# yanmin-wu/EDA

Hardware: AMD Instinct MI355X
Metric: scenes/sec fwd+bwd (50k pts, 256 queries, 80 tok) (higher is better)
Workload: dtype f32

## Files before the change

eda_amd/csrc/capi.hip:

```cpp
#include "eda_common.h"

#include <stdarg.h>

int g_eda_fma_mode = 0;

static thread_local char g_err[512] = "";

void eda_set_error(const char *fmt, ...) {
  va_list ap;
  va_start(ap, fmt);
  vsnprintf(g_err, sizeof(g_err), fmt, ap);
  va_end(ap);
}

extern "C" int eda_version(void) { return EDA_HIP_ABI_VERSION; }
extern "C" const char *eda_last_error_string(void) { return g_err; }
extern "C" int eda_set_fma_mode(int mode) {
  if (mode != 0 && mode != 1) {
    eda_set_error("eda_set_fma_mode: mode must be 0 or 1");
    return EDA_ERR_INVALID_ARG;
  }
  g_eda_fma_mode = mode;
  return 0;
}
extern "C" int eda_get_fma_mode(void) { return g_eda_fma_mode; }

#include <atomic>
#include <mutex>
#include <stdlib.h>
namespace {
struct KnobRow { const char *name; long dflt; };
const KnobRow kKnobs[EDA_K_COUNT] = {
    {"EDA_FPS_CU_RESERVE", 0},
    {"EDA_FPS_BUCKET", -1},
    {"EDA_FPS_BUCKET_NW", 16},
    {"EDA_FPS_SMALL_T", 512},
    {"EDA_FPS_SPEC", 1},
    {"EDA_FPS_T", 512},
    {"EDA_FPS_P", -1},
    {"EDA_FPS_TEST_GIVEUP", 0},
    {"EDA_BQ_SCAN", 0},
    {"EDA_GEMM_DBG", 0},
    {"EDA_GEMM_DMA", -1},
    {"EDA_GEMM_DMA_MAP", -1},
    {"EDA_GEMM_STREAM_GRID", 0},
    {"EDA_GEMM_STREAM_B3", 1},
    {"EDA_GEMM_STREAM", 1},
    {"EDA_GEMM_STREAM_MINR", 32768},
    {"EDA_GEMM_CFG", -1},
    {"EDA_GEMM_LN_BM", 0},
    {"EDA_GEMM_LN_VAR", 0},
    {"EDA_GEMM_SPLITK", -1},
    {"EDA_GEMM_KC96", -1},
    {"EDA_GEMM_B3ROWS", 1},
    {"EDA_FPS_BACKGROUND", 0},
    {"EDA_MHA2_PRIO", 1},
    {"EDA_MHA2_BWD_DBUF", 0},
    {"EDA_MHA2_BWD_MERGE", -1},
    {"EDA_MHA2_KSPLIT", -1},
    {"EDA_MHA4", 0},
    {"EDA_MHA3", 1},
    {"EDA_MHA3_DBG", 0},
    {"EDA_BN_SMALL_CQ", 4},
    {"EDA_SA_LAYER_FUSE", 1},
    {"EDA_SA_BNBWD_FUSE", 1},
    {"EDA_SA_BWD_B3", 1},
    {"EDA_WGRAD_BF16X3", 1},
    {"EDA_WGRAD_WGS", 144},
    {"EDA_DETERMINISTIC", 0},
    {"EDA_FROZEN_NW", 0},
    {"EDA_PEER_SPIN_LOG2", 24},
    {"EDA_PEER_ALLOC", 0},
};
EdaEnv g_env;
std::atomic<int> g_env_ready{0};
std::atomic<unsigned> g_env_epoch{1};
std::mutex g_env_mu;
void env_load(EdaEnv &e) {
  for (int k = 0; k < EDA_K_COUNT; ++k) {
    const char *s = getenv(kKnobs[k].name);
    e.set[k] = s && *s;
    e.val[k] = e.set[k] ? atol(s) : kKnobs[k].dflt;
  }
  e.skip_on = false; e.skip_k = e.skip_n = 0; e.skip_e = -1;
  if (const char *sk = getenv("EDA_GEMM_STREAM_SKIP"))
    e.skip_on = sscanf(sk, "%d,%d,%d", &e.skip_k, &e.skip_n, &e.skip_e) >= 2;
}
}
int g_eda_deterministic = -1;
const EdaEnv &eda_env() {
  if (!g_env_ready.load(std::memory_order_acquire)) {
    std::lock_guard<std::mutex> lock(g_env_mu);
    if (!g_env_ready.load(std::memory_order_relaxed)) { env_load(g_env); g_env_ready.store(1, std::memory_order_release); }
  }
  return g_env;
}
unsigned eda_env_epoch() { return g_env_epoch.load(std::memory_order_relaxed); }
void eda_fps_env_reset();
void eda_gemm_env_reset();
void eda_wgrad_env_reset();
extern "C" int eda_reload_env(void) {
  {
    std::lock_guard<std::mutex> lock(g_env_mu);
    env_load(g_env);
    g_env_ready.store(1, std::memory_order_release);
    g_env_epoch.fetch_add(1, std::memory_order_relaxed);
  }
  g_eda_deterministic = -1;
  eda_fps_env_reset(); eda_gemm_env_reset(); eda_wgrad_env_reset();
  return 0;
}
extern "C" int eda_set_deterministic(int on) {
  if (on != 0 && on != 1) { eda_set_error("eda_set_deterministic: 0 or 1"); return EDA_ERR_INVALID_ARG; }
  g_eda_deterministic = on;
  return 0;
}
extern "C" int eda_get_deterministic(void) { return eda_deterministic() ? 1 : 0; }

namespace {
__global__ __launch_bounds__(256) void zero_kernel(uint4 *p16, size_t n16, unsigned char *tail, size_t ntail) {
  const size_t i = (size_t)blockIdx.x * 256 + threadIdx.x;
  const size_t stride = (size_t)gridDim.x * 256;
  for (size_t k = i; k < n16; k += stride) p16[k] = make_uint4(0u, 0u, 0u, 0u);
  if (i < ntail) tail[i] = 0;
}
}

int eda_zero_async(void *ptr, size_t bytes, hipStream_t stream) {
  if (bytes == 0) return 0;
  unsigned char *p = reinterpret_cast<unsigned char *>(ptr);
  size_t head = (16 - (reinterpret_cast<uintptr_t>(p) & 15u)) & 15u;
  if (head > bytes) head = bytes;
  if (head) {
    hipLaunchKernelGGL(zero_kernel, dim3(1), dim3(256), 0, stream, nullptr, (size_t)0, p, head);
    p += head; bytes -= head;
  }
  const size_t n16 = bytes / 16, ntail = bytes % 16;
  size_t blocks = (n16 + 255) / 256;
  if (blocks > 4096) blocks = 4096;
  if (blocks < 1) blocks = 1;
  hipLaunchKernelGGL(zero_kernel, dim3((unsigned)blocks), dim3(256), 0, stream,
                     reinterpret_cast<uint4 *>(p), n16, p + n16 * 16, ntail);
  hipError_t e = hipGetLastError();
  if (e != hipSuccess) { eda_set_error("eda_zero_async: %s", hipGetErrorString(e)); return (int)e; }
  return 0;
// ... 133 lines not shown
```

eda_amd/csrc/eda_common.h:

```cpp
#pragma once
#include <hip/hip_runtime.h>
#include <stdint.h>
#include <stdio.h>

#include "../../include/eda_hip.h"

#define EDA_WAVE 64

void eda_set_error(const char *fmt, ...);
extern int g_eda_fma_mode;

enum EdaKnob : int {
  EDA_K_FPS_CU_RESERVE, EDA_K_FPS_BUCKET, EDA_K_FPS_BUCKET_NW, EDA_K_FPS_SMALL_T, EDA_K_FPS_SPEC, EDA_K_FPS_T, EDA_K_FPS_P,
  EDA_K_FPS_TEST_GIVEUP, EDA_K_BQ_SCAN, EDA_K_GEMM_DBG, EDA_K_GEMM_DMA, EDA_K_GEMM_DMA_MAP, EDA_K_GEMM_STREAM_GRID,
  EDA_K_GEMM_STREAM_B3, EDA_K_GEMM_STREAM, EDA_K_GEMM_STREAM_MINR, EDA_K_GEMM_CFG, EDA_K_GEMM_LN_BM, EDA_K_GEMM_LN_VAR,
  EDA_K_GEMM_SPLITK, EDA_K_GEMM_KC96, EDA_K_GEMM_B3ROWS, EDA_K_FPS_BACKGROUND, EDA_K_MHA2_PRIO, EDA_K_MHA2_BWD_DBUF, EDA_K_MHA2_BWD_MERGE, EDA_K_MHA2_KSPLIT, EDA_K_MHA4, EDA_K_MHA3, EDA_K_MHA3_DBG, EDA_K_BN_SMALL_CQ, EDA_K_SA_LAYER_FUSE, EDA_K_SA_BNBWD_FUSE,
  EDA_K_SA_BWD_B3, EDA_K_WGRAD_BF16X3, EDA_K_WGRAD_WGS, EDA_K_DETERMINISTIC, EDA_K_FROZEN_NW, EDA_K_PEER_SPIN_LOG2, EDA_K_PEER_ALLOC, EDA_K_COUNT
};
struct EdaEnv {
  long val[EDA_K_COUNT];
  bool set[EDA_K_COUNT];
  int skip_k, skip_n, skip_e;
  bool skip_on;
};
const EdaEnv &eda_env();
unsigned eda_env_epoch();
static inline long eda_knob(EdaKnob k) { return eda_env().val[k]; }
static inline bool eda_knob_set(EdaKnob k) { return eda_env().set[k]; }
extern int g_eda_deterministic;
static inline bool eda_deterministic() { return (g_eda_deterministic < 0 ? eda_knob(EDA_K_DETERMINISTIC) : g_eda_deterministic) != 0; }

#define EDA_CHECK_ARG(cond, msg)                         \
  do {                                                   \
    if (!(cond)) {                                       \
      eda_set_error("%s: %s", __func__, msg);            \
      return EDA_ERR_INVALID_ARG;                        \
    }                                                    \
  } while (0)

#include <mutex>
#include <set>
#include <utility>
static inline hipError_t eda_set_max_dynamic_lds(const void *kern, size_t bytes) {
  static std::mutex mu;
  static std::set<std::pair<const void *, int>> done;
  int dev = 0;
  hipError_t e = hipGetDevice(&dev);
  if (e != hipSuccess) return e;
  std::lock_guard<std::mutex> lock(mu);
  if (done.count({kern, dev})) return hipSuccess;
  e = hipFuncSetAttribute(kern, hipFuncAttributeMaxDynamicSharedMemorySize, (int)bytes);
  if (e == hipSuccess) done.insert({kern, dev});
  return e;
}

#define EDA_CHECK_LAUNCH()                                              \
  do {                                                                  \
    hipError_t e__ = hipGetLastError();                                 \
    if (e__ != hipSuccess) {                                            \
      eda_set_error("%s: launch failed: %s", __func__,                  \
                    hipGetErrorString(e__));                            \
      return (int)e__;                                                  \
    }                                                                   \
  } while (0)

#define EDA_CHECK_HIP(expr)                                             \
  do {                                                                  \
    hipError_t e__ = (expr);                                            \
    if (e__ != hipSuccess) {                                            \
      eda_set_error("%s: %s failed: %s", __func__, #expr,               \
                    hipGetErrorString(e__));                            \
      return (int)e__;                                                  \
    }                                                                   \
  } while (0)

template <int MODE>
__device__ __forceinline__ float eda_sumsq3(float a, float b, float c) {
  if (MODE == 0) {
    float t = b * b;
    t = __builtin_fmaf(a, a, t);
    t = __builtin_fmaf(c, c, t);
    return t;
  } else {
    return (a * a + b * b) + c * c;
  }
}

#define EDA_DPP_QUAD_XOR1 0xB1
#define EDA_DPP_QUAD_XOR2 0x4E
#define EDA_DPP_ROW_ROR(n) (0x120 + (n))

template <int CTRL>
__device__ __forceinline__ int eda_dpp(int v) {
  return __builtin_amdgcn_update_dpp(v, v, CTRL, 0xF, 0xF, false);
}

__device__ __forceinline__ int eda_row_max_i32(int v) {
  v = max(v, eda_dpp<EDA_DPP_QUAD_XOR1>(v));
  v = max(v, eda_dpp<EDA_DPP_QUAD_XOR2>(v));
// ... 62 lines not shown
```

eda_amd/csrc/mha2.h:

```cpp
#pragma once
#include <hip/hip_runtime.h>

struct Mha2Args {
  const float *q, *k, *v;
  long q_sb, q_sl, k_sb, k_sl, v_sb, v_sl;
  float *o; long o_sb, o_sl;
  float *lse;
  const unsigned char *mask;
  int B, H, Lq, Lk;
  float scale, p_drop;
  const unsigned long long *seed_ptr; unsigned salt;
  const float *dout; long do_sb, do_sl;
  float *dq, *dk, *dv;
  long dq_sb, dq_sl, dk_sb, dk_sl, dv_sb, dv_sl;
  int n_kb;
  int n_qs;
  int q_per_wg;
  int prio_mode;
  int dtype;
  float *dq_part;
  float *dkv_part;
  int bwd_merge;
  unsigned *bwd_tickets;
  const float *xq; long xq_sb, xq_sl;
  const float *wq; long ldwq;
  const float *bq;
  float *q_out; long qo_sb, qo_sl;
  int n_ksplit, keys_per_split;
  int dbg3;
  float *fwd_part;
  unsigned *fwd_tickets;
};

int eda_mha2_fwd_launch(Mha2Args &a, void *ws, size_t ws_bytes, hipStream_t stream);
size_t eda_mha2_fwd_workspace_bytes(int B, int H, int Lq, int Lk);
int eda_mha3_fwd_launch(Mha2Args &a, hipStream_t stream);
bool eda_mha4_takes(int dtype, int Lq, int Lk);
size_t eda_mha4_fwd_workspace_bytes(int B, int H, int Lq, int Lk);
int eda_mha4_fwd_launch(Mha2Args &a, void *ws, size_t ws_bytes, hipStream_t stream);
int eda_mha2_qproj_fwd_launch(Mha2Args &a, hipStream_t stream);
int eda_mha2_bwd_launch(Mha2Args &a, void *ws, size_t ws_bytes, unsigned *tickets, size_t tickets_bytes, hipStream_t stream);
size_t eda_mha2_bwd_workspace_bytes(int B, int H, int Lq, int Lk);
size_t eda_mha2_bwd_ticket_bytes(int B, int H, int Lq, int Lk);
```

eda_amd/csrc/mha2.hip:

```cpp
#include "eda_common.h"
#include "mha2.h"

#include <stdlib.h>

namespace {

constexpr int HD = 36;
constexpr int KSTEPS = 9;
constexpr float LOG2E = 1.4426950408889634f;
constexpr float LN2 = 0.6931471805599453f;

typedef float f32x4 __attribute__((ext_vector_type(4)));
typedef unsigned u32x2 __attribute__((ext_vector_type(2)));

#ifdef EDA_MHA2_PROFILE
__device__ unsigned long long mha2_prof[64 * 8];
#define PSTAMP(slot)                                                   \
  do {                                                                 \
    __builtin_amdgcn_sched_barrier(0);                                 \
    const unsigned long long now__ = __builtin_amdgcn_s_memtime();     \
    asm volatile("s_waitcnt lgkmcnt(0)" ::"s"(now__));                 \
    prof_acc[slot] += now__ - prof_t;                                  \
    prof_t = now__;                                                    \
    __builtin_amdgcn_sched_barrier(0);                                 \
// ... 1172 lines not shown
      a.n_ksplit = sp.ns;
      const int chunks = (a.Lk + FWD_SPLIT_CHK - 1) / FWD_SPLIT_CHK;
      a.keys_per_split = (chunks + sp.ns - 1) / sp.ns * FWD_SPLIT_CHK;
      const bool one = a.keys_per_split == FWD_SPLIT_CHK;
      return one ? launch_fwd<4, 4, FWD_SPLIT_CHK, 1, true>(a, stream) : launch_fwd<4, 4, FWD_SPLIT_CHK, 2, true>(a, stream);
    }
  }
  {
    const int rc3 = eda_mha3_fwd_launch(a, stream);
    if (rc3 >= 0) return rc3;
  }
  const bool short_q = (long)BH * ((a.Lq + 255) / 256) < 192;
  if (a.Lk <= 144) {
    if (short_q) return launch_fwd<4, 2, 192, 1>(a, stream);
    return launch_fwd<16, 1, 192, 1>(a, stream);
  }
  if (a.Lk <= 256) {
    if (short_q) return launch_fwd<4, 4, 256, 1>(a, stream);
    return launch_fwd<16, 1, 256, 1>(a, stream);
  }
  if (short_q) return launch_fwd<4, 4, 256, 2>(a, stream);
  return launch_fwd<16, 1, 256, 2>(a, stream);
}

int eda_mha2_qproj_fwd_launch(Mha2Args &a, hipStream_t stream) {
  if (a.B == 0 || a.Lq == 0) return 0;
  const dim3 g((unsigned)(a.B * a.H * ((a.Lq + 63) / 64))), b(256);
  const bool drop = a.p_drop > 0.f;
#define EDA_QP(AR)                                                                                   \
  do {                                                                                               \
    if (drop) hipLaunchKernelGGL((mha2_qproj_fwd_kernel<true, AR>), g, b, 0, stream, a);             \
    else hipLaunchKernelGGL((mha2_qproj_fwd_kernel<false, AR>), g, b, 0, stream, a);                 \
  } while (0)
  if (a.dtype == EDA_DTYPE_BF16) EDA_QP(ArBf16);
  else if (a.dtype == EDA_DTYPE_F16) EDA_QP(ArFp16);
  else EDA_QP(ArF32);
#undef EDA_QP
  EDA_CHECK_LAUNCH();
  return 0;
}

#ifdef EDA_MHA2_PROFILE
extern "C" int eda_mha2_profile_read(unsigned long long *out16) {
  static unsigned long long all[64 * 8], zero[64 * 8];
  if (hipMemcpyFromSymbol(all, HIP_SYMBOL(mha2_prof), sizeof(all)) != hipSuccess) return 1;
  for (int i = 0; i < 16; ++i) out16[i] = 0;
  for (int s = 0; s < 64; ++s)
    for (int i = 0; i < 8; ++i) out16[i] += all[s * 8 + i];
  return hipMemcpyToSymbol(HIP_SYMBOL(mha2_prof), zero, sizeof(zero)) != hipSuccess;
}
#endif

size_t eda_mha2_bwd_ticket_bytes(int B, int H, int Lq, int Lk) {
  if (B <= 0 || Lq <= 0 || Lk <= 0) return 0;
  return (sizeof(unsigned) * bwd_ticket_words(bwd_plan(B, H, Lq, Lk), B, H) + 255) / 256 * 256;
}
size_t eda_mha2_bwd_workspace_bytes(int B, int H, int Lq, int Lk) {
  if (B <= 0 || Lq <= 0 || Lk <= 0) return 0;
  return eda_mha2_bwd_ticket_bytes(B, H, Lq, Lk) + sizeof(float) * bwd_workspace_floats(bwd_plan(B, H, Lq, Lk), B, H, Lq, Lk);
}

int eda_mha2_bwd_launch(Mha2Args &a, void *ws, size_t ws_bytes, unsigned *tickets, size_t tickets_bytes, hipStream_t stream) {
  if (a.B == 0) return 0;
  a.prio_mode = (int)eda_knob(EDA_K_MHA2_PRIO);
  const BwdPlan p = bwd_plan(a.B, a.H, a.Lq, a.Lk);
  a.n_kb = p.n_kb; a.n_qs = p.n_qs; a.q_per_wg = p.q_per_wg;
  const size_t tk = eda_mha2_bwd_ticket_bytes(a.B, a.H, a.Lq, a.Lk);
  const size_t need = tk + sizeof(float) * bwd_workspace_floats(p, a.B, a.H, a.Lq, a.Lk);
  EDA_CHECK_ARG(need == 0 || (ws && ws_bytes >= need && (reinterpret_cast<uintptr_t>(ws) & 15u) == 0),
                "workspace of eda_mha_bwd_workspace_bytes() required (16-byte aligned)");
  EDA_CHECK_ARG(!tickets || tickets_bytes >= tk, "ticket buffer of eda_mha_bwd_ticket_bytes() required");
  float *w = reinterpret_cast<float *>(reinterpret_cast<unsigned char *>(ws) + tk);
  a.dq_part = nullptr; a.dkv_part = nullptr; a.bwd_tickets = nullptr;
  if (p.n_kb > 1) { a.dq_part = w; w += (size_t)p.n_kb * a.B * a.Lq * a.H * HD; }
  if (p.n_qs > 1) a.dkv_part = w;
  if (tk) {
    a.bwd_tickets = tickets ? tickets : reinterpret_cast<unsigned *>(ws);
    if (!tickets)
      if (int rc = eda_zero_async(ws, tk, stream)) return rc;
  }
  a.bwd_merge = p.merge;
  const bool dbuf = eda_knob(EDA_K_MHA2_BWD_DBUF) != 0;
  int rc;
  if (p.variant == 0) rc = launch_bwd<16, 1, 64, 2>(a, stream);
  else if (p.variant == 1) rc = dbuf ? launch_bwd<9, 1, 64, 2>(a, stream) : launch_bwd<9, 1, 64, 1>(a, stream);
  else rc = dbuf ? launch_bwd<5, 3, 96, 2>(a, stream) : launch_bwd<5, 3, 96, 1>(a, stream);
  if (rc || p.merge) return rc;
  const int D = a.H * HD;
  if (p.n_kb > 1) {
    const long items = (long)a.B * a.Lq * D / 4;
    hipLaunchKernelGGL(mha2_part_reduce_kernel, dim3((unsigned)((items + 255) / 256)), dim3(256), 0, stream,
                       a.dq_part, p.n_kb, 1, a.B, a.Lq, D, a.dq, a.dq_sb, a.dq_sl, a.dq, a.dq_sb, a.dq_sl);
    EDA_CHECK_LAUNCH();
  }
  if (p.n_qs > 1) {
    const long items = 2L * a.B * a.Lk * D / 4;
    hipLaunchKernelGGL(mha2_part_reduce_kernel, dim3((unsigned)((items + 255) / 256)), dim3(256), 0, stream,
                       a.dkv_part, p.n_qs, 2, a.B, a.Lk, D, a.dk, a.dk_sb, a.dk_sl, a.dv, a.dv_sb, a.dv_sl);
    EDA_CHECK_LAUNCH();
  }
  return 0;
}

namespace {

bool mult4(long v) { return (v & 3) == 0; }
bool al16(const void *p) { return (reinterpret_cast<uintptr_t>(p) & 15u) == 0; }

__global__ __launch_bounds__(256) void mha2_fill_rows_kernel(float *__restrict__ o, long sb, long sl, int B, int L, int D,
                                                             float value) {
  const long i = (long)blockIdx.x * 256 + threadIdx.x;
  if (i >= (long)B * L * D) return;
  const long row = i / D;
  const int col = (int)(i - row * D);
  const long bb = row / L, l = row - bb * L;
  o[bb * sb + l * sl + col] = value;
}
int fill_rows(float *o, long sb, long sl, int B, int L, int D, float value, hipStream_t stream) {
  const long n = (long)B * L * D;
  if (n <= 0) return 0;
  hipLaunchKernelGGL(mha2_fill_rows_kernel, dim3((unsigned)((n + 255) / 256)), dim3(256), 0, stream, o, sb, sl, B, L, D, value);
  EDA_CHECK_LAUNCH();
  return 0;
}

}

extern "C" size_t eda_mha_fwd_workspace_bytes(int B, int H, int Lq, int Lk) { return eda_mha2_fwd_workspace_bytes(B, H, Lq, Lk); }

extern "C" int eda_mha_fwd(const float *q, const float *k, const float *v, long q_sb, long q_sl, long k_sb, long k_sl,
                           long v_sb, long v_sl, const unsigned char *key_padding_mask, int B, int H, int Lq, int Lk,
                           int head_dim, float scale, float p_drop, const unsigned long long *seed_ptr, unsigned salt,
                           float *out, float *lse, int dtype, void *stream_) {
  return eda_mha_fwd_ws(q, k, v, q_sb, q_sl, k_sb, k_sl, v_sb, v_sl, key_padding_mask, B, H, Lq, Lk, head_dim, scale, p_drop,
                        seed_ptr, salt, out, lse, dtype, nullptr, 0, stream_);
}

extern "C" int eda_mha_fwd_ws(const float *q, const float *k, const float *v, long q_sb, long q_sl, long k_sb, long k_sl,
                              long v_sb, long v_sl, const unsigned char *key_padding_mask, int B, int H, int Lq, int Lk,
                              int head_dim, float scale, float p_drop, const unsigned long long *seed_ptr, unsigned salt,
                              float *out, float *lse, int dtype, void *ws, size_t ws_bytes, void *stream_) {
  hipStream_t stream = (hipStream_t)stream_;
  EDA_CHECK_ARG(dtype == EDA_DTYPE_F32 || dtype == EDA_DTYPE_BF16 || dtype == EDA_DTYPE_F16,
                "dtype must be EDA_DTYPE_F32 / BF16 / F16");
  EDA_CHECK_ARG(head_dim == HD, "only head_dim 36 (d_model 288 / 8 heads) is built");
  EDA_CHECK_ARG(B >= 0 && H > 0 && Lq >= 0 && Lk >= 0, "bad dimension");
  if (B == 0 || Lq == 0) return 0;
  EDA_CHECK_ARG(q && k && v && out && lse, "null pointer");
  EDA_CHECK_ARG(p_drop >= 0.f && p_drop < 1.f && (p_drop == 0.f || seed_ptr), "bad dropout arguments");
  EDA_CHECK_ARG(mult4(q_sb) && mult4(q_sl) && mult4(k_sb) && mult4(k_sl) && mult4(v_sb) && mult4(v_sl) &&
                    al16(q) && al16(k) && al16(v) && al16(out),
                "rows must be 16-byte aligned");
  EDA_CHECK_ARG((long)B * H <= 65535, "B*H too large");
  if (Lk == 0) {
    if (int rc = fill_rows(out, (long)Lq * H * HD, (long)H * HD, B, Lq, H * HD, 0.f, stream)) return rc;
    return fill_rows(lse, (long)H * Lq, (long)Lq, B, H, Lq, -INFINITY, stream);
  }
  Mha2Args m = {};
  m.q = q; m.k = k; m.v = v; m.q_sb = q_sb; m.q_sl = q_sl; m.k_sb = k_sb; m.k_sl = k_sl;
  m.v_sb = v_sb; m.v_sl = v_sl; m.o = out; m.o_sb = (long)Lq * H * HD; m.o_sl = (long)H * HD;
  m.lse = lse; m.mask = key_padding_mask; m.B = B; m.H = H; m.Lq = Lq; m.Lk = Lk; m.scale = scale;
  m.p_drop = p_drop; m.seed_ptr = seed_ptr; m.salt = salt; m.dtype = dtype;
  return eda_mha2_fwd_launch(m, ws, ws_bytes, stream);
}

extern "C" int eda_mha_qproj_supported(int H, int head_dim, int Lk) { return H * head_dim == QP_D && head_dim == HD && Lk >= 1 && Lk <= 192; }

// ... 107 lines not shown
```

Measured before the change: 464.4.

## Add MFMA-based bf16x3 split-precision attention backward kernel for variant 0

Adds a new attention backward kernel (mha3_bwd) that splits f32 Q/K/V/dO into three bf16 planes and computes the score and gradient products with 16x16x32 bf16 MFMA using six-product emulation. It stages Q/dO/O chunks into LDS via global_load_lds and overlaps conversion of the next chunk with the dQ phase on separate waves. It is enabled by default for the variant-0 config and falls back to the old path when shapes do not fit. The aim is to replace the slower f32 backward, at the cost of bf16x3 precision emulation and heavy LDS use that limits occupancy.

After: 469.3, median of 6. 1.01x the previous value.

```diff
diff --git a/eda_amd/csrc/capi.hip b/eda_amd/csrc/capi.hip
--- a/eda_amd/csrc/capi.hip
+++ b/eda_amd/csrc/capi.hip
@@ -61,6 +61,7 @@
     {"EDA_MHA4", 0},
     {"EDA_MHA3", 1},
     {"EDA_MHA3_DBG", 0},
+    {"EDA_MHA3_BWD", 1},
     {"EDA_BN_SMALL_CQ", 4},
     {"EDA_SA_LAYER_FUSE", 1},
     {"EDA_SA_BNBWD_FUSE", 1},
diff --git a/eda_amd/csrc/eda_common.h b/eda_amd/csrc/eda_common.h
--- a/eda_amd/csrc/eda_common.h
+++ b/eda_amd/csrc/eda_common.h
@@ -14,7 +14,7 @@
   EDA_K_FPS_CU_RESERVE, EDA_K_FPS_BUCKET, EDA_K_FPS_BUCKET_NW, EDA_K_FPS_SMALL_T, EDA_K_FPS_SPEC, EDA_K_FPS_T, EDA_K_FPS_P,
   EDA_K_FPS_TEST_GIVEUP, EDA_K_BQ_SCAN, EDA_K_GEMM_DBG, EDA_K_GEMM_DMA, EDA_K_GEMM_DMA_MAP, EDA_K_GEMM_STREAM_GRID,
   EDA_K_GEMM_STREAM_B3, EDA_K_GEMM_STREAM, EDA_K_GEMM_STREAM_MINR, EDA_K_GEMM_CFG, EDA_K_GEMM_LN_BM, EDA_K_GEMM_LN_VAR,
-  EDA_K_GEMM_SPLITK, EDA_K_GEMM_KC96, EDA_K_GEMM_B3ROWS, EDA_K_FPS_BACKGROUND, EDA_K_MHA2_PRIO, EDA_K_MHA2_BWD_DBUF, EDA_K_MHA2_BWD_MERGE, EDA_K_MHA2_KSPLIT, EDA_K_MHA4, EDA_K_MHA3, EDA_K_MHA3_DBG, EDA_K_BN_SMALL_CQ, EDA_K_SA_LAYER_FUSE, EDA_K_SA_BNBWD_FUSE,
+  EDA_K_GEMM_SPLITK, EDA_K_GEMM_KC96, EDA_K_GEMM_B3ROWS, EDA_K_FPS_BACKGROUND, EDA_K_MHA2_PRIO, EDA_K_MHA2_BWD_DBUF, EDA_K_MHA2_BWD_MERGE, EDA_K_MHA2_KSPLIT, EDA_K_MHA4, EDA_K_MHA3, EDA_K_MHA3_DBG, EDA_K_MHA3_BWD, EDA_K_BN_SMALL_CQ, EDA_K_SA_LAYER_FUSE, EDA_K_SA_BNBWD_FUSE,
   EDA_K_SA_BWD_B3, EDA_K_WGRAD_BF16X3, EDA_K_WGRAD_WGS, EDA_K_DETERMINISTIC, EDA_K_FROZEN_NW, EDA_K_PEER_SPIN_LOG2, EDA_K_PEER_ALLOC, EDA_K_COUNT
 };
 struct EdaEnv {
diff --git a/eda_amd/csrc/mha2.h b/eda_amd/csrc/mha2.h
--- a/eda_amd/csrc/mha2.h
+++ b/eda_amd/csrc/mha2.h
@@ -39,6 +39,7 @@
 size_t eda_mha4_fwd_workspace_bytes(int B, int H, int Lq, int Lk);
 int eda_mha4_fwd_launch(Mha2Args &a, void *ws, size_t ws_bytes, hipStream_t stream);
 int eda_mha2_qproj_fwd_launch(Mha2Args &a, hipStream_t stream);
+int eda_mha3_bwd_launch(Mha2Args &a, hipStream_t stream);
 int eda_mha2_bwd_launch(Mha2Args &a, void *ws, size_t ws_bytes, unsigned *tickets, size_t tickets_bytes, hipStream_t stream);
 size_t eda_mha2_bwd_workspace_bytes(int B, int H, int Lq, int Lk);
 size_t eda_mha2_bwd_ticket_bytes(int B, int H, int Lq, int Lk);
diff --git a/eda_amd/csrc/mha2.hip b/eda_amd/csrc/mha2.hip
--- a/eda_amd/csrc/mha2.hip
+++ b/eda_amd/csrc/mha2.hip
@@ -1278,7 +1278,10 @@
   a.bwd_merge = p.merge;
   const bool dbuf = eda_knob(EDA_K_MHA2_BWD_DBUF) != 0;
   int rc;
-  if (p.variant == 0) rc = launch_bwd<16, 1, 64, 2>(a, stream);
+  if (p.variant == 0) {
+    rc = eda_mha3_bwd_launch(a, stream);
+    if (rc < 0) rc = launch_bwd<16, 1, 64, 2>(a, stream);
+  }
   else if (p.variant == 1) rc = dbuf ? launch_bwd<9, 1, 64, 2>(a, stream) : launch_bwd<9, 1, 64, 1>(a, stream);
   else rc = dbuf ? launch_bwd<5, 3, 96, 2>(a, stream) : launch_bwd<5, 3, 96, 1>(a, stream);
   if (rc || p.merge) return rc;
diff --git a/eda_amd/csrc/mha3_bwd.hip b/eda_amd/csrc/mha3_bwd.hip
--- /dev/null
+++ b/eda_amd/csrc/mha3_bwd.hip
@@ -0,0 +1,547 @@
+#include "eda_common.h"
+#include "mha2.h"
+
+namespace {
+
+constexpr int HD = 36;
+constexpr float LOG2E = 1.4426950408889634f;
+constexpr int NW = 16, NT = NW * 64;
+constexpr int KB = 16 * NW;
+constexpr int QC = 32;
+constexpr int KROW = 40;
+constexpr int KREM = 24;
+constexpr int TROW = QC + 8;
+constexpr int DROW = KB + 8;
+constexpr int NPB = 6;
+
+typedef float f32x4 __attribute__((ext_vector_type(4)));
+typedef float f32x2 __attribute__((ext_vector_type(2)));
+typedef __bf16 bf16x2 __attribute__((ext_vector_type(2)));
+typedef __bf16 bf16x8 __attribute__((ext_vector_type(8)));
+typedef unsigned u32x2 __attribute__((ext_vector_type(2)));
+typedef unsigned u32x4 __attribute__((ext_vector_type(4)));
+
+constexpr int STG_B = QC * HD * 4;
+constexpr int RP_B = QC * KROW * 2;
+constexpr int RR_B = QC * KREM * 2;
+constexpr int TP_B = 32 * TROW * 2;
+constexpr int TR_B = 16 * TROW * 2;
+constexpr int DP_B = QC * DROW * 2;
+constexpr int KP_B = 32 * DROW * 2;
+constexpr int KR_B = 16 * DROW * 2;
+constexpr int O_STG = 0;
+constexpr int O_QP = O_STG + 3 * STG_B, O_QR = O_QP + 3 * RP_B;
+constexpr int O_EP = O_QR + RR_B, O_ER = O_EP + 3 * RP_B;
+constexpr int O_QT = O_ER + RR_B, O_QTR = O_QT + 3 * TP_B;
+constexpr int O_ET = O_QTR + TR_B, O_ETR = O_ET + 3 * TP_B;
+constexpr int O_DS = O_ETR + TR_B;
+constexpr int O_KT = O_DS + 3 * DP_B, O_KTR = O_KT + 3 * KP_B;
+constexpr int O_LSE = O_KTR + KR_B, O_DEL = O_LSE + QC * 4;
+constexpr int LDS_BYTES = O_DEL + QC * 4;
+static_assert(LDS_BYTES <= 160 * 1024, "LDS budget");
+static_assert(O_QP % 16 == 0 && O_EP % 16 == 0 && O_QT % 16 == 0 && O_ET % 16 == 0 && O_DS % 16 == 0 && O_KT % 16 == 0 &&
+              O_KTR % 16 == 0 && O_QTR % 16 == 0 && O_ETR % 16 == 0 && O_QR % 16 == 0 && O_ER % 16 == 0, "alignment");
+
+__device__ __forceinline__ unsigned hash32(unsigned x) {
+  x ^= x >> 16; x *= 0x7feb352dU; x ^= x >> 15; x *= 0x846ca68bU; x ^= x >> 16;
+  return x;
+}
+__device__ __forceinline__ float grp_sum(float v) {
+  u32x2 r = __builtin_amdgcn_permlane32_swap(__float_as_uint(v), __float_as_uint(v), false, false);
+  v = __uint_as_float(r.x) + __uint_as_float(r.y);
+  r = __builtin_amdgcn_permlane16_swap(__float_as_uint(v), __float_as_uint(v), false, false);
+  return __uint_as_float(r.x) + __uint_as_float(r.y);
+}
+__device__ __forceinline__ f32x4 grp_sum4(f32x4 v) {
+  f32x4 r;
+  r[0] = grp_sum(v[0]); r[1] = grp_sum(v[1]); r[2] = grp_sum(v[2]); r[3] = grp_sum(v[3]);
+  return r;
+}
+
+__device__ __forceinline__ void split2(float a, float b, unsigned (&pl)[3]) {
+  const bf16x2 h = __builtin_convertvector(f32x2{a, b}, bf16x2);
+  pl[0] = __builtin_bit_cast(unsigned, h);
+  const float ra = a - (float)h[0], rb = b - (float)h[1];
+  const bf16x2 m = __builtin_convertvector(f32x2{ra, rb}, bf16x2);
+  pl[1] = __builtin_bit_cast(unsigned, m);
+  const bf16x2 l = __builtin_convertvector(f32x2{ra - (float)m[0], rb - (float)m[1]}, bf16x2);
+  pl[2] = __builtin_bit_cast(unsigned, l);
+}
+
+__device__ __forceinline__ f32x4 mma32(u32x4 a, u32x4 b, f32x4 c) {
+  return __builtin_amdgcn_mfma_f32_16x16x32_bf16(__builtin_bit_cast(bf16x8, a), __builtin_bit_cast(bf16x8, b), c, 0, 0, 0);
+}
+__device__ __forceinline__ f32x4 prod6(const u32x4 (&a)[3], const u32x4 (&b)[3], f32x4 acc) {
+  f32x4 s = mma32(a[1], b[1], f32x4{0, 0, 0, 0});
+  acc = mma32(a[0], b[2], acc);
+  s = mma32(a[2], b[0], s);
+  acc = mma32(a[1], b[0], acc);
+  s = mma32(a[0], b[1], s);
+  acc = mma32(a[0], b[0], acc);
+  return acc + s;
+}
+
+struct DropCfg { unsigned seed, thresh; float inv_keep; };
+
+__device__ __forceinline__ void row_planes(const float *row, float mul, bool valid, int g, u32x4 (&pl)[3], u32x4 &rem) {
+  float4 x = make_float4(0.f, 0.f, 0.f, 0.f), y = x, z = x;
+  if (valid) {
+    x = *reinterpret_cast<const float4 *>(row + 8 * g);
+    y = *reinterpret_cast<const float4 *>(row + 8 * g + 4);
+    z = *reinterpret_cast<const float4 *>(row + 32);
+  }
+  const float v8[8] = {x.x * mul, x.y * mul, x.z * mul, x.w * mul, y.x * mul, y.y * mul, y.z * mul, y.w * mul};
+#pragma unroll
+  for (int i = 0; i < 4; ++i) {
+    unsigned w[3];
+    split2(v8[2 * i], v8[2 * i + 1], w);
+#pragma unroll
+    for (int p = 0; p < 3; ++p) pl[p][i] = w[p];
+  }
+  unsigned r01[3], r23[3];
+  split2(z.x * mul, z.y * mul, r01);
+  split2(z.z * mul, z.w * mul, r23);
+  const int pb = g == 1 ? 2 : 1;
+  rem = g < 3 ? u32x4{r01[0], r23[0], r01[pb], r23[pb]} : u32x4{0u, 0u, 0u, 0u};
+}
+
+template <bool DROP>
+__global__ __launch_bounds__(NT) void mha3_bwd_kernel(const Mha2Args a) {
+  extern __shared__ __attribute__((aligned(16))) unsigned char smem[];
+  float *stg = reinterpret_cast<float *>(smem + O_STG);
+  float *lse_s = reinterpret_cast<float *>(smem + O_LSE);
+  float *del_s = reinterpret_cast<float *>(smem + O_DEL);
+
+  const int tid = threadIdx.x, lane = tid & 63;
+  const int wave = __builtin_amdgcn_readfirstlane(tid >> 6);
+  const int g = lane >> 4, c = lane & 15;
+  const int BH = a.B * a.H;
+  const int bh = (int)(blockIdx.x % (unsigned)BH);
+  const int rest = (int)(blockIdx.x / (unsigned)BH);
+  const int kb = rest % a.n_kb, qsp = rest / a.n_kb;
+  const int b = bh / a.H, h = bh - b * a.H;
+  const int ks = wave;
+
+  const int kblock0 = kb * KB;
+  const int key0 = kblock0 + 16 * ks;
+  const bool wave_live = key0 < a.Lk;
+  const int nks_live = min(NW, (a.Lk - kblock0 + 15) >> 4);
+  const int ki = key0 + c;
+  const bool kvalid = ki < a.Lk;
+  const bool kdead = !kvalid || (a.mask && a.mask[(long)b * a.Lk + (kvalid ? ki : 0)]);
+
+  DropCfg dc = {0u, 0u, 1.f};
+  if (DROP && a.p_drop > 0.f) {
+    dc.seed = hash32((unsigned)(*a.seed_ptr) * 0x9E3779B1u + a.salt);
+    dc.thresh = (unsigned)((double)a.p_drop * 65536.0 + 0.5);
+    dc.inv_keep = 1.f / (1.f - a.p_drop);
+  }
+
+  for (int i = tid; i < 3 * DP_B / 4; i += NT) reinterpret_cast<unsigned *>(smem + O_DS)[i] = 0u;
+  for (int i = tid; i < 4 * TROW / 2; i += NT) {
+    reinterpret_cast<unsigned *>(smem + O_QTR + 12 * TROW * 2)[i] = 0u;
+    reinterpret_cast<unsigned *>(smem + O_ETR + 12 * TROW * 2)[i] = 0u;
+  }
+  for (int i = tid; i < 4 * DROW / 2; i += NT) reinterpret_cast<unsigned *>(smem + O_KTR + 12 * DROW * 2)[i] = 0u;
+  const float *kbase = a.k + (long)b * a.k_sb + h * HD;
+  for (int i = tid; i < (KB / 2) * HD; i += NT) {
+    const int kq = i / HD, d = i - kq * HD;
+    const int k0 = kblock0 + 2 * kq;
+    const float x0 = k0 < a.Lk ? kbase[(long)k0 * a.k_sl + d] : 0.f;
+    const float x1 = k0 + 1 < a.Lk ? kbase[(long)(k0 + 1) * a.k_sl + d] : 0.f;
+    unsigned pl[3];
+    split2(x0, x1, pl);
+    if (d < 32) {
+#pragma unroll
+      for (int p = 0; p < 3; ++p) *reinterpret_cast<unsigned *>(smem + O_KT + p * KP_B + (d * DROW + 2 * kq) * 2) = pl[p];
+    } else {
+#pragma unroll
+      for (int p = 0; p < 3; ++p) *reinterpret_cast<unsigned *>(smem + O_KTR + ((4 * p + d - 32) * DROW + 2 * kq) * 2) = pl[p];
+    }
+  }
+  u32x4 kp[3], kx, vp[3], vx;
+  {
+    const int kr = min(ki, a.Lk - 1);
+    const bool ld = wave_live && kvalid;
+    row_planes(kbase + (long)kr * a.k_sl, 1.f, ld, g, kp, kx);
+    row_planes(a.v + (long)b * a.v_sb + (long)kr * a.v_sl + h * HD, dc.inv_keep, ld, g, vp, vx);
+  }
+
+  const int qbeg = qsp * a.q_per_wg;
+  const int qend = min(a.Lq, qbeg + a.q_per_wg);
+  const float *qbase = a.q + (long)b * a.q_sb + h * HD;
+  const float *dbase = a.dout + (long)b * a.do_sb + h * HD;
+  const float *obase = a.o + (long)b * a.o_sb + h * HD;
+  const float sl2 = a.scale * LOG2E;
+  const int D = a.H * HD;
+  float *dq_out = a.dq + (long)b * a.dq_sb + h * HD;
+  long dq_sl = a.dq_sl;
+  if (a.n_kb > 1) { dq_out = a.dq_part + ((long)kb * a.B + b) * a.Lq * D + h * HD; dq_sl = D; }
+  const __amdgpu_buffer_rsrc_t rs_dq = __builtin_amdgcn_make_buffer_rsrc(dq_out, 0, a.Lq * D * 4, 0x00020000);
+
+  auto stage = [&](int q0) {
+    constexpr int G = QC * 9, P = (G + 63) / 64;
+    for (int pc = wave; pc < 3 * P; pc += NW) {
+      const int t = pc / P, pp = pc - t * P;
+      const int i = 64 * pp + lane;
+      if (G % 64 == 0 || i < G) {
+        const int row = i / 9, c4 = i - row * 9;
+        const int grow = min(q0 + row, a.Lq - 1);
+        const float *src = t == 0 ? qbase + (long)grow * a.q_sl : (t == 1 ? dbase + (long)grow * a.do_sl : obase + (long)grow * a.o_sl);
+        __builtin_amdgcn_global_load_lds((const __attribute__((address_space(1))) void *)(src + 4 * c4),
+                                         (__attribute__((address_space(3))) void *)(stg + t * (QC * HD) + 256 * pp), 16, 0, 0);
+      }
+    }
+  };
+
+  auto convert = [&](int q0, int w0, int nw) {
+    const int nthr = 64 * nw;
+    int t0 = tid - 64 * w0;
+    asm volatile("" : "+v"(t0));
+    if (t0 < QC * 8) {
+      const int row = t0 >> 3, sub = t0 & 7;
+      const int gr = min(q0 + row, a.Lq - 1);
+      const float ls = a.lse[(long)bh * a.Lq + gr];
+      const float *dr = stg + QC * HD + row * HD, *orow = stg + 2 * QC * HD + row * HD;
+      const float4 d4 = *reinterpret_cast<const float4 *>(dr + 4 * sub), o4 = *reinterpret_cast<const float4 *>(orow + 4 * sub);
+      float part = d4.x * o4.x + d4.y * o4.y + d4.z * o4.z + d4.w * o4.w;
+      if (sub == 0) {
+        const float4 d8 = *reinterpret_cast<const float4 *>(dr + 32), o8 = *reinterpret_cast<const float4 *>(orow + 32);
+        part += d8.x * o8.x + d8.y * o8.y + d8.z * o8.z + d8.w * o8.w;
+      }
+      part += __shfl_xor(part, 1);
+      part += __shfl_xor(part, 2);
+      part += __shfl_xor(part, 4);
+      if (sub == 0) {
+        const bool valid = q0 + row < qend;
+        lse_s[row] = valid ? ls * LOG2E : INFINITY;
+        del_s[row] = valid ? part : 0.f;
+      }
+    }
+    for (int i = t0; i < 2 * (QC / 2) * 18; i += nthr) {
+      const int t = i / ((QC / 2) * 18), r = i - t * ((QC / 2) * 18);
+      const int qq = r / 18, dp = r - qq * 18;
+      const float *src = stg + t * (QC * HD) + 2 * qq * HD + 2 * dp;
+      const float2 x0 = *reinterpret_cast<const float2 *>(src), x1 = *reinterpret_cast<const float2 *>(src + HD);
+      unsigned pa[3], pb[3];
+      split2(x0.x, x0.y, pa);
+      split2(x1.x, x1.y, pb);
+      unsigned char *rp = smem + (t ? O_EP : O_QP), *rr = smem + (t ? O_ER : O_QR);
+      unsigned char *tp = smem + (t ? O_ET : O_QT), *tr = smem + (t ? O_ETR : O_QTR);
+      if (dp < 16) {
+#pragma unroll
+        for (int p = 0; p < 3; ++p) {
+          *reinterpret_cast<unsigned *>(rp + p * RP_B + ((2 * qq) * KROW + 2 * dp) * 2) = pa[p];
+          *reinterpret_cast<unsigned *>(rp + p * RP_B + ((2 * qq + 1) * KROW + 2 * dp) * 2) = pb[p];
+        }
+      } else {
+        const int o = dp - 16;
+        unsigned *r0 = reinterpret_cast<unsigned *>(rr + (2 * qq) * KREM * 2) + o;
+        unsigned *r1 = reinterpret_cast<unsigned *>(rr + (2 * qq + 1) * KREM * 2) + o;
+        r0[0] = pa[0]; r0[2] = pa[0]; r0[4] = pa[1]; r0[6] = pa[0]; r0[8] = pa[2]; r0[10] = pa[1];
+        r1[0] = pb[0]; r1[2] = pb[0]; r1[4] = pb[1]; r1[6] = pb[0]; r1[8] = pb[2]; r1[10] = pb[1];
+      }
+#pragma unroll
+      for (int p = 0; p < 3; ++p) {
+        const unsigned lo = (pa[p] & 0xffffu) | (pb[p] << 16);
+        const unsigned hi = (pa[p] >> 16) | (pb[p] & 0xffff0000u);
+        const int d = 2 * dp;
+        unsigned char *base = d < 32 ? tp + p * TP_B + d * TROW * 2 : tr + (4 * p + d - 32) * TROW * 2;
+        *reinterpret_cast<unsigned *>(base + 4 * qq) = lo;
+        *reinterpret_cast<unsigned *>(base + TROW * 2 + 4 * qq) = hi;
+      }
+    }
+  };
+
+  f32x4 dk[3] = {{0, 0, 0, 0}, {0, 0, 0, 0}, {0, 0, 0, 0}};
+  f32x4 dv[3] = {{0, 0, 0, 0}, {0, 0, 0, 0}, {0, 0, 0, 0}};
+
+  auto trow = [&](const unsigned char *p, int c, int g) {
+    const unsigned char *row = p + (c * TROW + 4 * g) * 2;
+    const u32x2 lo = *reinterpret_cast<const u32x2 *>(row), hi = *reinterpret_cast<const u32x2 *>(row + 32);
+    return u32x4{lo.x, lo.y, hi.x, hi.y};
+  };
+
+  auto phase_a = [&](int q0) {
+    if (!wave_live) return;
+    int ln = lane;
+    asm volatile("" : "+v"(ln));
+    const int c = ln & 15, g = ln >> 4;
+    const int nsub = min(2, (qend - q0 + 15) >> 4);
+    float pd[2][4], ds[2][4];
+#pragma unroll
+    for (int j = 0; j < 2; ++j) {
+      if (j < nsub) {
+        f32x4 sacc, pacc;
+        {
+          u32x4 qa[3], ea[3];
+#pragma unroll
+          for (int p = 0; p < 3; ++p) {
+            qa[p] = *reinterpret_cast<const u32x4 *>(smem + O_QP + p * RP_B + ((16 * j + c) * KROW + 8 * g) * 2);
+            ea[p] = *reinterpret_cast<const u32x4 *>(smem + O_EP + p * RP_B + ((16 * j + c) * KROW + 8 * g) * 2);
+          }
+          u32x4 qx = {0u, 0u, 0u, 0u}, ex = {0u, 0u, 0u, 0u};
+          if (g < 3) {
+            qx = *reinterpret_cast<const u32x4 *>(smem + O_QR + ((16 * j + c) * KREM + 8 * g) * 2);
+            ex = *reinterpret_cast<const u32x4 *>(smem + O_ER + ((16 * j + c) * KREM + 8 * g) * 2);
+          }
+          sacc = prod6(qa, kp, mma32(qx, kx, f32x4{0, 0, 0, 0}));
+          pacc = prod6(ea, vp, mma32(ex, vx, f32x4{0, 0, 0, 0}));
+        }
+        const float4 lse4 = *reinterpret_cast<const float4 *>(lse_s + 16 * j + 4 * g);
+        const float4 del4 = *reinterpret_cast<const float4 *>(del_s + 16 * j + 4 * g);
+        const float lse_r[4] = {lse4.x, lse4.y, lse4.z, lse4.w};
+        const float del_r[4] = {del4.x, del4.y, del4.z, del4.w};
+        unsigned h16[4] = {0xffffu, 0xffffu, 0xffffu, 0xffffu};
+        if (DROP) {
+          const int odd = c & 1;
+          const unsigned qa0 = (unsigned)(q0 + 16 * j + 4 * g + 2 * odd);
+          const unsigned kev = (unsigned)(ki & ~1);
+          const unsigned hx = hash32(dc.seed ^ (((unsigned)bh * (unsigned)a.Lq + qa0) * (unsigned)a.Lk + kev));
+          const unsigned hy = hash32(dc.seed ^ (((unsigned)bh * (unsigned)a.Lq + qa0 + 1u) * (unsigned)a.Lk + kev));
+          const unsigned nx = (unsigned)__builtin_amdgcn_mov_dpp((int)hx, 0xB1, 0xf, 0xf, true);
+          const unsigned ny = (unsigned)__builtin_amdgcn_mov_dpp((int)hy, 0xB1, 0xf, 0xf, true);
+          const unsigned h0 = odd ? nx : hx, h1 = odd ? ny : hy, h2 = odd ? hx : nx, h3 = odd ? hy : ny;
+          const int sh = 16 * odd;
+          h16[0] = (h0 >> sh) & 0xffffu; h16[1] = (h1 >> sh) & 0xffffu;
+          h16[2] = (h2 >> sh) & 0xffffu; h16[3] = (h3 >> sh) & 0xffffu;
+        }
+#pragma unroll
+        for (int r = 0; r < 4; ++r) {
+          float p = __builtin_amdgcn_exp2f(__builtin_fmaf(sacc[r], sl2, -lse_r[r]));
+          p = kdead ? 0.f : p;
+          float dp = pacc[r], pk = p;
+          if (DROP) {
+            const bool keep = h16[r] >= dc.thresh;
+            dp = keep ? dp : 0.f;
+            pk = keep ? p : 0.f;
+          }
+          pd[j][r] = pk;
+          ds[j][r] = p * (dp - del_r[r]);
+        }
+      } else {
+#pragma unroll
+        for (int r = 0; r < 4; ++r) { pd[j][r] = 0.f; ds[j][r] = 0.f; }
+      }
+    }
+    auto planes = [&](const float (&x)[2][4], u32x4 (&pl)[3], bool to_tile) {
+#pragma unroll
+      for (int j = 0; j < 2; ++j)
+#pragma unroll
+        for (int r2 = 0; r2 < 2; ++r2) {
+          unsigned w[3];
+          split2(x[j][2 * r2], x[j][2 * r2 + 1], w);
+#pragma unroll
+          for (int p = 0; p < 3; ++p) pl[p][2 * j + r2] = w[p];
+          if (to_tile && j < nsub) {
+            unsigned short *dst = reinterpret_cast<unsigned short *>(smem + O_DS) + (16 * j + 4 * g + 2 * r2) * DROW + 16 * ks + c;
+#pragma unroll
+            for (int p = 0; p < 3; ++p) {
+              dst[p * (DP_B / 2)] = (unsigned short)(w[p] & 0xffffu);
+              dst[p * (DP_B / 2) + DROW] = (unsigned short)(w[p] >> 16);
+            }
+          }
+        }
+    };
+    auto accumulate = [&](int o_t, int o_tr, const u32x4 (&pl)[3], f32x4 (&acc)[3]) {
+#pragma unroll
+      for (int t = 0; t < 2; ++t) {
+        u32x4 xa[3];
+#pragma unroll
+        for (int p = 0; p < 3; ++p) xa[p] = trow(smem + o_t + p * TP_B + 16 * t * TROW * 2, c, g);
+        acc[t] = prod6(xa, pl, acc[t]);
+      }
+      const u32x4 xx = trow(smem + o_tr, c, g);
+#pragma unroll
+      for (int p = 2; p >= 0; --p) acc[2] = mma32(xx, pl[p], acc[2]);
+    };
+    {
+      u32x4 pp[3];
+      planes(pd, pp, false);
+      accumulate(O_ET, O_ETR, pp, dv);
+    }
+    {
+      u32x4 sp[3];
+      planes(ds, sp, true);
+      accumulate(O_QT, O_QTR, sp, dk);
+    }
+  };
+
+  auto phase_b = [&](int q0, int item) {
+    const int nsub = min(2, (qend - q0 + 15) >> 4);
+    const bool full = item < 4;
+    const int j = full ? item >> 1 : item - 4, n = full ? item & 1 : 2;
+    if (j >= nsub) return;
+    int ln = lane;
+    asm volatile("" : "+v"(ln));
+    const int c = ln & 15, g = ln >> 4;
+    const int nsl = (nks_live + 1) >> 1;
+    const unsigned char *dsr = smem + O_DS + ((16 * j + c) * DROW + 8 * g) * 2;
+    const unsigned char *ktr = full ? smem + O_KT + ((16 * n + c) * DROW + 8 * g) * 2 : smem + O_KTR + (c * DROW + 8 * g) * 2;
+    auto slice = [&](int s, f32x4 acc) {
+      u32x4 sb[3];
+#pragma unroll
+      for (int p = 0; p < 3; ++p) sb[p] = *reinterpret_cast<const u32x4 *>(dsr + p * DP_B + 64 * s);
+      if (full) {
+        u32x4 ka[3];
+#pragma unroll
+        for (int p = 0; p < 3; ++p) ka[p] = *reinterpret_cast<const u32x4 *>(ktr + p * KP_B + 64 * s);
+        return prod6(ka, sb, acc);
+      }
+      const u32x4 kx_ = *reinterpret_cast<const u32x4 *>(ktr + 64 * s);
+      acc = mma32(kx_, sb[2], acc); acc = mma32(kx_, sb[1], acc);
+      return mma32(kx_, sb[0], acc);
+    };
+    f32x4 acc0 = {0, 0, 0, 0}, acc1 = {0, 0, 0, 0};
+    if (nsl == KB / 32) {
+#pragma unroll
+      for (int s = 0; s < KB / 32; s += 2) { acc0 = slice(s, acc0); acc1 = slice(s + 1, acc1); }
+    } else {
+      int s = 0;
+      for (; s + 1 < nsl; s += 2) { acc0 = slice(s, acc0); acc1 = slice(s + 1, acc1); }
+      if (s < nsl) acc0 = slice(s, acc0);
+    }
+    f32x4 r = acc0 + acc1;
+    if (!full) r = grp_sum4(r);
+    const int gq = q0 + 16 * j + c;
+    if (gq < qend && (full || g == 0)) {
+      const float sc = a.scale;
+      const f32x4 val = {r[0] * sc, r[1] * sc, r[2] * sc, r[3] * sc};
+      if (a.n_kb > 1 && a.bwd_merge)
+        __builtin_amdgcn_raw_buffer_store_b128(__builtin_bit_cast(u32x4, val), rs_dq, (gq * D + 16 * n + 4 * g) * 4, 0, 16);
+      else
+        *reinterpret_cast<f32x4 *>(dq_out + (long)gq * dq_sl + 16 * n + 4 * g) = val;
+    }
+  };
+
+  const int nchunks = qend > qbeg ? (qend - qbeg + QC - 1) / QC : 0;
+  if (nchunks > 0) stage(qbeg);
+  EDA_SYNC_DMA();
+  if (nchunks > 0) convert(qbeg, 0, NW);
+  __syncthreads();
+  if (nchunks > 1) stage(qbeg + QC);
+  for (int ci = 0; ci < nchunks; ++ci) {
+    const int q0 = qbeg + ci * QC;
+    phase_a(q0);
+    EDA_SYNC_DMA();
+    if (wave < NPB) phase_b(q0, wave);
+    else if (ci + 1 < nchunks) convert(q0 + QC, NPB, NW - NPB);
+    __syncthreads();
+    if (ci + 2 < nchunks) stage(q0 + 2 * QC);
+  }
+
+  if (wave_live) { dk[2] = grp_sum4(dk[2]); dv[2] = grp_sum4(dv[2]); }
+  const long kv_per = (long)a.B * a.Lk * D;
+  if (kvalid && wave_live) {
+    const float sc = a.scale, ik = dc.inv_keep;
+    if (a.n_qs > 1 && a.bwd_merge) {
+      const __amdgpu_buffer_rsrc_t rk = __builtin_amdgcn_make_buffer_rsrc(
+          a.dkv_part + (long)qsp * 2 * kv_per + ((long)b * a.Lk + ki) * D + h * HD, 0, HD * 4, 0x00020000);
+      const __amdgpu_buffer_rsrc_t rv = __builtin_amdgcn_make_buffer_rsrc(
+          a.dkv_part + (long)qsp * 2 * kv_per + kv_per + ((long)b * a.Lk + ki) * D + h * HD, 0, HD * 4, 0x00020000);
+      __builtin_amdgcn_raw_buffer_store_b128(__builtin_bit_cast(u32x4, dk[0] * sc), rk, 16 * g, 0, 16);
+      __builtin_amdgcn_raw_buffer_store_b128(__builtin_bit_cast(u32x4, dk[1] * sc), rk, 64 + 16 * g, 0, 16);
+      __builtin_amdgcn_raw_buffer_store_b128(__builtin_bit_cast(u32x4, dv[0] * ik), rv, 16 * g, 0, 16);
+      __builtin_amdgcn_raw_buffer_store_b128(__builtin_bit_cast(u32x4, dv[1] * ik), rv, 64 + 16 * g, 0, 16);
+      if (g == 0) {
+        __builtin_amdgcn_raw_buffer_store_b128(__builtin_bit_cast(u32x4, dk[2] * sc), rk, 128, 0, 16);
+        __builtin_amdgcn_raw_buffer_store_b128(__builtin_bit_cast(u32x4, dv[2] * ik), rv, 128, 0, 16);
+      }
+    } else {
+      float *ok = a.dk + (long)b * a.dk_sb + (long)ki * a.dk_sl + h * HD;
+      float *ov = a.dv + (long)b * a.dv_sb + (long)ki * a.dv_sl + h * HD;
+      if (a.n_qs > 1) {
+        ok = a.dkv_part + (long)qsp * 2 * kv_per + ((long)b * a.Lk + ki) * D + h * HD;
+        ov = ok + kv_per;
+      }
+      *reinterpret_cast<f32x4 *>(ok + 4 * g) = dk[0] * sc;
+      *reinterpret_cast<f32x4 *>(ok + 16 + 4 * g) = dk[1] * sc;
+      *reinterpret_cast<f32x4 *>(ov + 4 * g) = dv[0] * ik;
+      *reinterpret_cast<f32x4 *>(ov + 16 + 4 * g) = dv[1] * ik;
+      if (g == 0) {
+        *reinterpret_cast<f32x4 *>(ok + 32) = dk[2] * sc;
+        *reinterpret_cast<f32x4 *>(ov + 32) = dv[2] * ik;
+      }
+    }
+  }
+  if (a.bwd_merge && (a.n_kb > 1 || a.n_qs > 1)) {
+    asm volatile("s_waitcnt vmcnt(0)" ::: "memory");
+    __syncthreads();
+    unsigned *flag = reinterpret_cast<unsigned *>(lse_s);
+    if (tid == 0) {
+      unsigned lq = 0u, lkv = 0u;
+      if (a.n_kb > 1) {
+        unsigned *tk = a.bwd_tickets + (long)bh * a.n_qs + qsp;
+        lq = __hip_atomic_fetch_add(tk, 1u, __ATOMIC_RELAXED, __HIP_MEMORY_SCOPE_AGENT) == (unsigned)a.n_kb - 1u;
+        if (lq) __hip_atomic_store(tk, 0u, __ATOMIC_RELAXED, __HIP_MEMORY_SCOPE_AGENT);
+      }
+      if (a.n_qs > 1) {
+        unsigned *tk = a.bwd_tickets + (long)BH * a.n_qs + (long)bh * a.n_kb + kb;
+        lkv = __hip_atomic_fetch_add(tk, 1u, __ATOMIC_RELAXED, __HIP_MEMORY_SCOPE_AGENT) == (unsigned)a.n_qs - 1u;
+        if (lkv) __hip_atomic_store(tk, 0u, __ATOMIC_RELAXED, __HIP_MEMORY_SCOPE_AGENT);
+      }
+      flag[0] = lq; flag[1] = lkv;
+    }
+    __syncthreads();
+    constexpr int MU = 4;
+    auto merge = [&](const float *p0, long zstride, int nz, int rows, int row0, float *fin, long fin_sl, int span_bytes) {
+      const int nitems = rows * 9;
+      for (int base = tid; base < nitems; base += NT * MU) {
+        f32x4 t[MU];
+        int off[MU];
+#pragma unroll
+        for (int u = 0; u < MU; ++u) {
+          const int i = min(base + u * NT, nitems - 1);
+          const int row = i / 9, c4 = i - row * 9;
+          off[u] = ((row0 + row) * D + 4 * c4) * 4;
+          t[u] = f32x4{0.f, 0.f, 0.f, 0.f};
+        }
+#pragma unroll 4
+        for (int z = 0; z < nz; ++z) {
+          const __amdgpu_buffer_rsrc_t rp = __builtin_amdgcn_make_buffer_rsrc(const_cast<float *>(p0 + z * zstride), 0, span_bytes, 0x00020000);
+#pragma unroll
+          for (int u = 0; u < MU; ++u) t[u] += __builtin_bit_cast(f32x4, __builtin_amdgcn_raw_buffer_load_b128(rp, off[u], 0, 16));
+        }
+#pragma unroll
+        for (int u = 0; u < MU; ++u) {
+          const int i = base + u * NT;
+          if (i < nitems) {
+            const int row = i / 9, c4 = i - row * 9;
+            *reinterpret_cast<f32x4 *>(fin + (long)(row0 + row) * fin_sl + 4 * c4) = t[u];
+          }
+        }
+      }
+    };
+    if (flag[0])
+      merge(a.dq_part + (long)b * a.Lq * D + h * HD, (long)a.B * a.Lq * D, a.n_kb, qend - qbeg, qbeg,
+            a.dq + (long)b * a.dq_sb + h * HD, a.dq_sl, a.Lq * D * 4);
+    if (flag[1]) {
+      const int nkeys = min(KB, a.Lk - kblock0);
+      const float *p0 = a.dkv_part + (long)b * a.Lk * D + h * HD;
+      merge(p0, 2 * kv_per, a.n_qs, nkeys, kblock0, a.dk + (long)b * a.dk_sb + h * HD, a.dk_sl, a.Lk * D * 4);
+      merge(p0 + kv_per, 2 * kv_per, a.n_qs, nkeys, kblock0, a.dv + (long)b * a.dv_sb + h * HD, a.dv_sl, a.Lk * D * 4);
+    }
+  }
+}
+
+}
+
+int eda_mha3_bwd_launch(Mha2Args &a, hipStream_t stream) {
+  if (eda_knob(EDA_K_MHA3_BWD) == 0) return -1;
+  if (a.dtype != EDA_DTYPE_F32 || a.Lk < 512 || a.Lq < 192) return -1;
+  if (a.q_per_wg % QC != 0 || (a.Lk + KB - 1) / KB != a.n_kb) return -1;
+  const dim3 grid((unsigned)(a.B * a.H * a.n_kb * a.n_qs)), block(NT);
+  hipError_t e;
+  if (a.p_drop > 0.f) {
+    auto kern = mha3_bwd_kernel<true>;
+    e = eda_set_max_dynamic_lds(reinterpret_cast<const void *>(kern), LDS_BYTES);
+    if (e == hipSuccess) hipLaunchKernelGGL(kern, grid, block, LDS_BYTES, stream, a);
+  } else {
+    auto kern = mha3_bwd_kernel<false>;
+    e = eda_set_max_dynamic_lds(reinterpret_cast<const void *>(kern), LDS_BYTES);
+    if (e == hipSuccess) hipLaunchKernelGGL(kern, grid, block, LDS_BYTES, stream, a);
+  }
+  if (e != hipSuccess) { eda_set_error("mha3_bwd: LDS attribute: %s", hipGetErrorString(e)); return (int)e; }
+  EDA_CHECK_LAUNCH();
+  return 0;
+}
```
